# soedinglab/MMseqs2

Measured on AMD Instinct MI355X. Metric: sw_gcells_per_s, higher is better.
Workload: dtype int16

## Files before the change

### mmseqs2_amd/csrc/sw_body.h

```cpp
#pragma once
#include "mmgpu_internal.h"
#include "pf_device.h"

namespace mmgpu {

namespace {

constexpr int GROUP = 16;
constexpr int WAVES = 4;
constexpr int GROUPS_PER_WAVE = 64 / GROUP;
constexpr int HITS_PER_WAVE = 2 * GROUPS_PER_WAVE;
constexpr unsigned NEG2 = 0x80008000u;

typedef short s16x2 __attribute__((ext_vector_type(2)));
typedef unsigned short u16x2 __attribute__((ext_vector_type(2)));

__device__ __forceinline__ unsigned pk_add_sat(unsigned a, unsigned b) {
    return __builtin_bit_cast(unsigned, __builtin_elementwise_add_sat(__builtin_bit_cast(s16x2, a),
                                                                      __builtin_bit_cast(s16x2, b)));
}
__device__ __forceinline__ unsigned pk_max_s(unsigned a, unsigned b) {
    return __builtin_bit_cast(unsigned, __builtin_elementwise_max(__builtin_bit_cast(s16x2, a),
                                                                  __builtin_bit_cast(s16x2, b)));
}
__device__ __forceinline__ unsigned pk_max_u(unsigned a, unsigned b) {
    return __builtin_bit_cast(unsigned, __builtin_elementwise_max(__builtin_bit_cast(u16x2, a),
                                                                  __builtin_bit_cast(u16x2, b)));
}
__device__ __forceinline__ unsigned pk_sub_sat_u(unsigned a, unsigned b) {
    return __builtin_bit_cast(unsigned, __builtin_elementwise_sub_sat(__builtin_bit_cast(u16x2, a),
                                                                      __builtin_bit_cast(u16x2, b)));
}
__device__ __forceinline__ unsigned bfi(unsigned mask, unsigned a, unsigned b) {
    return (a & mask) | (b & ~mask);
}

constexpr int SW_HALF_LIMIT = 2048 - 256;
constexpr int SW_HALF_MAX_GAP = 2048;
constexpr int SW_HALF_MARK = -1;
typedef _Float16 h16x2 __attribute__((ext_vector_type(2)));
__device__ __forceinline__ h16x2 as_h(unsigned a) { return __builtin_bit_cast(h16x2, a); }
__device__ __forceinline__ unsigned as_u(h16x2 a) { return __builtin_bit_cast(unsigned, a); }
__device__ __forceinline__ unsigned h_add(unsigned a, unsigned b) { return as_u(as_h(a) + as_h(b)); }
__device__ __forceinline__ unsigned h_sub(unsigned a, unsigned b) { return as_u(as_h(a) - as_h(b)); }
__device__ __forceinline__ unsigned h_max(unsigned a, unsigned b) {
    return as_u(__builtin_elementwise_maximum(as_h(a), as_h(b)));
}
__device__ __forceinline__ unsigned h_max3(unsigned a, unsigned b, unsigned c) {
    return as_u(__builtin_elementwise_maximum(__builtin_elementwise_maximum(as_h(a), as_h(b)), as_h(c)));
}
__device__ __forceinline__ unsigned short h_bits(int v) { return __builtin_bit_cast(unsigned short, (_Float16)v); }
__device__ __forceinline__ int h_value(unsigned bits) { return (int)(float)__builtin_bit_cast(_Float16, (unsigned short)bits); }
__device__ __forceinline__ unsigned from_lane_above(unsigned head, unsigned v) {
    return __builtin_amdgcn_update_dpp(head, v, 0x111 , 0xF, 0xF, false);
}
__device__ __forceinline__ unsigned from_lane_above_or_zero(unsigned v) {
    return __builtin_amdgcn_update_dpp(0u, v, 0x111 , 0xF, 0xF, true);
}

#ifndef MMGPU_SW_PREFETCH
#define MMGPU_SW_PREFETCH 1
#endif
#define SW_KEEP_IN_ROW(x) asm volatile("" : "+v"(x))

template <int R>
struct Tile {
    static constexpr int ROWS = GROUP * R;
    static constexpr int LANE_STRIDE = lane_stride_bytes(R);
    static constexpr int ROW_STRIDE = GROUP * LANE_STRIDE;
};
static_assert(GROUP == 16, "sw_profile_bytes and sw_tiles (mmgpu_internal.h) assume 16-lane groups");

template <int R, bool REV, bool HALF = false>
__device__ __forceinline__ void build_profile(unsigned char *lds, const uint8_t *q, const int8_t *cb, int qlen,
                                              int tile_base, const int8_t *mat, int alphabet, const int8_t *prof) {
    using T = Tile<R>;
    const int total = (alphabet + 1) * T::ROWS;
    for (int idx = threadIdx.x; idx < total; idx += blockDim.x) {
        const int letter = idx / T::ROWS;
        const int row = idx - letter * T::ROWS;
        const int rg = tile_base + row;
        short v = (short)-32768;
        if (letter < alphabet && rg < qlen) {
            const int qi = REV ? (qlen - 1 - rg) : rg;
            v = prof ? (short)prof[letter * qlen + qi] : (short)((int)mat[letter * alphabet + q[qi]] + (int)cb[qi]);
        }
        const int lane = row / R, r = row - lane * R;
        if constexpr (HALF) v = (short)h_bits(v);
        *reinterpret_cast<short *>(lds + letter * T::ROW_STRIDE + lane * T::LANE_STRIDE + r * 2) = v;
    }
}

__device__ __forceinline__ bool sw_rev_wanted(const SwLaunch &L, uint32_t slot, int min_start) {
    const mmgpu_sw_hit &f = L.out[slot];
    const int s = f.score;
    if (L.rev_mode == 2) return s > 0 && L.rev_force[slot] != 0;
    return s > 0 && s >= min_start && !(L.rev_mode == 1 && f.word != 0);
}

constexpr int SW_REV_JOB_HITS = 1024;
static_assert(SW_REV_JOB_HITS == SW_REV_JOB_MAX, "host and kernel disagree on the reverse job size");
static_assert(SW_LDS_HEADER == SW_REV_JOB_HITS * 2 + 64, "the header holds the live hits and the scheduling words");
constexpr int SW_HALF_FLAG_AT = SW_REV_JOB_HITS * 2 + 20;
__device__ __forceinline__ uint32_t sw_half_any_marked() {
    extern __shared__ __attribute__((aligned(16))) unsigned char lds_all[];
    return *reinterpret_cast<const uint32_t *>(lds_all + SW_HALF_FLAG_AT);
}

template <int R, bool MULTI, bool REV, bool PF, bool HALF = false, bool MARKED = false>
__device__ __forceinline__ void sw_body(const SwLaunch &L, const SwJob job) {
    static_assert(!(HALF || MARKED) || (!MULTI && !REV && !(HALF && MARKED)), "f16 and its int16 re-run: single-tile forward scans");
    constexpr bool PACKED = REV || MARKED;
    using T = Tile<R>;
    extern __shared__ __attribute__((aligned(16))) unsigned char lds_all[];
    uint16_t *live = reinterpret_cast<uint16_t *>(lds_all);
    uint32_t *live_wave = reinterpret_cast<uint32_t *>(lds_all + SW_REV_JOB_HITS * 2);
    uint32_t *next_chunk = reinterpret_cast<uint32_t *>(lds_all + SW_REV_JOB_HITS * 2 + 16);
    uint32_t *half_flag = reinterpret_cast<uint32_t *>(lds_all + SW_HALF_FLAG_AT);
    unsigned char *lds = lds_all + SW_LDS_HEADER;
    if (MULTI) __builtin_amdgcn_s_setprio(3);
    const int lane = threadIdx.x & 63;
    const int wave = __builtin_amdgcn_readfirstlane(threadIdx.x >> 6);
    const int g = lane & (GROUP - 1);
    const int grp = lane / GROUP;

    const uint32_t qbeg = L.q_off[job.query];
    const int qlen = (int)(L.q_off[job.query + 1] - qbeg);
    const uint8_t *q = L.q_res + qbeg;
    const int8_t *cb = L.q_cb + qbeg;
    const int qbias = L.q_bias[job.query];
    const int8_t *prof = nullptr;
    if (L.q_prof_off) {
        const uint32_t po = L.q_prof_off[job.query];
        if (po != 0xFFFFFFFFu) prof = L.q_prof + po;
    }
    const int n_tiles = MULTI ? (int)sw_tiles((uint32_t)qlen, R) : 1;
    const uint32_t tile_bytes = sw_profile_bytes(R, L.alphabet);
    const bool resident = MULTI && sw_multi_resident((uint32_t)n_tiles, R, L.alphabet, L.resident_lds);
    const bool dynamic = !MULTI || resident;
    auto build_all_tiles = [&]() {
        for (int tile = 0; tile < n_tiles; ++tile)
            build_profile<R, REV>(lds + (uint32_t)tile * tile_bytes, q, cb, qlen, tile * T::ROWS, L.mat, L.alphabet, prof);
        __syncthreads();
    };

    const unsigned go2 = (HALF ? (unsigned)h_bits(L.gap_open) : (unsigned)L.gap_open) * 0x10001u;
    const unsigned ge2 = (HALF ? (unsigned)h_bits(L.gap_extend) : (unsigned)L.gap_extend) * 0x10001u;
    const unsigned pad_letter = (unsigned)L.alphabet;

    if (threadIdx.x == 0) *next_chunk = 0;
    if (HALF && threadIdx.x == 0) *half_flag = 0;
    if (!MULTI && !PACKED) {
        build_profile<R, REV, HALF>(lds, q, cb, qlen, 0, L.mat, L.alphabet, prof);
        __syncthreads();
    }
    if (MULTI && !REV && resident) build_all_tiles();

    uint32_t n_hits = job.hit_end - job.hit_begin;
    if (PACKED) {
        const int min_start = REV ? L.q_minstart[job.query] : 0;
        uint32_t total = 0;
        for (uint32_t base = 0; base < n_hits; base += WAVES * 64) {
            const uint32_t idx = base + threadIdx.x;
            bool pass = false;
            if (idx < n_hits) {
                const uint32_t slot = L.hit_out[job.hit_begin + idx];
                pass = MARKED ? L.out[slot].score == SW_HALF_MARK : sw_rev_wanted(L, slot, min_start);
            }
            const unsigned long long bal = __ballot(pass);
            if (lane == 0) live_wave[wave] = (uint32_t)__popcll(bal);
            __syncthreads();
            uint32_t before = 0, round_total = 0;
#pragma unroll
            for (int w = 0; w < WAVES; ++w) {
                const uint32_t c = live_wave[w];
                before += w < wave ? c : 0u;
                round_total += c;
            }
            if (pass) live[total + before + (uint32_t)__popcll(bal & ((1ull << lane) - 1ull))] = (uint16_t)idx;
            total += round_total;
            __syncthreads();
        }
        n_hits = total;
        if (n_hits == 0) return;
        if (!MULTI) {
            build_profile<R, REV>(lds, q, cb, qlen, 0, L.mat, L.alphabet, prof);
            __syncthreads();
        }
        if (MULTI && resident) build_all_tiles();
    }
    const uint32_t n_iter = (n_hits + WAVES * HITS_PER_WAVE - 1) / (WAVES * HITS_PER_WAVE);

    for (uint32_t it = 0; dynamic || it < n_iter; ++it) {
        uint32_t chunk = it * WAVES + wave;
        if (dynamic) {
            if (lane == 0) chunk = atomicAdd(next_chunk, 1u);
            chunk = __builtin_amdgcn_readfirstlane(chunk);
        }
        const uint32_t slot0 = chunk * HITS_PER_WAVE;
        if (dynamic && slot0 >= n_hits) break;

        const uint32_t sA = slot0 + grp * 2, sB = sA + 1;
        const bool vA = sA < n_hits, vB = sB < n_hits;
        const uint32_t hA = job.hit_begin + (PACKED ? (uint32_t)live[vA ? sA : 0] : sA);
        const uint32_t hB = job.hit_begin + (PACKED ? (uint32_t)live[vB ? sB : 0] : sB);
        const uint32_t tA = vA ? L.hit_target[hA] : 0u, tB = vB ? L.hit_target[hB] : 0u;
        const uint8_t *pA = L.t_res + (size_t)L.t_off4[tA] * 4;
        const uint8_t *pB = L.t_res + (size_t)L.t_off4[tB] * 4;
        int colsA = vA ? (int)L.t_len[tA] : 0, colsB = vB ? (int)L.t_len[tB] : 0;
        int r0A = 0, r0B = 0;
        int endA = 0, endB = 0;
        unsigned rev_target = 0xFFFFFFFFu;
        if (REV) {
            mmgpu_sw_hit fa, fb;
            fa.score = 0; fa.q_end = 0; fa.t_end = 0;
            fb = fa;
            if (vA) fa = L.out[L.hit_out[hA]];
            if (vB) fb = L.out[L.hit_out[hB]];
            colsA = vA ? fa.t_end + 1 : 0;
            colsB = vB ? fb.t_end + 1 : 0;
            endA = colsA > 0 ? fa.t_end : 0;
            endB = colsB > 0 ? fb.t_end : 0;
            r0A = colsA > 0 ? qlen - 1 - fa.q_end : 0;
            r0B = colsB > 0 ? qlen - 1 - fb.q_end : 0;
            rev_target = (colsA > 0 ? (unsigned)fa.score & 0xFFFFu : 0xFFFFu) | ((colsB > 0 ? (unsigned)fb.score & 0xFFFFu : 0xFFFFu) << 16);
        }
        int ncols = colsA > colsB ? colsA : colsB;
        ncols = max(ncols, __shfl_xor(ncols, 16));
        ncols = max(ncols, __shfl_xor(ncols, 32));
        ncols = __builtin_amdgcn_readfirstlane(ncols);
        const int nsteps = ncols + GROUP - 1;
        int mincols = colsA < colsB ? colsA : colsB;
        mincols = min(mincols, __shfl_xor(mincols, 16));
        mincols = min(mincols, __shfl_xor(mincols, 32));
        mincols = __builtin_amdgcn_readfirstlane(mincols);

        unsigned long long bestA = 0, bestB = 0;

        uint2 *scr = nullptr;
        unsigned scr_grp = 0;
        if (MULTI) {
            scr = L.scratch + (size_t)((job.shape >> 8) * WAVES + wave) * GROUPS_PER_WAVE * 2 * L.scratch_cols;
            scr_grp = (unsigned)grp * 2u * L.scratch_cols;
        }

        for (int tile = 0; tile < n_tiles; ++tile) {
            const int tile_base = tile * T::ROWS;
            if (MULTI && !resident) {
                __syncthreads();
                build_profile<R, REV>(lds, q, cb, qlen, tile_base, L.mat, L.alphabet, prof);
                __syncthreads();
            }
            const unsigned char *const lds_tile = MULTI && resident ? lds + (uint32_t)tile * tile_bytes : lds;
            const uint2 *scr_in = MULTI ? scr + (size_t)((tile + 1) & 1) * L.scratch_cols : nullptr;
            uint2 *scr_out = MULTI ? scr + (size_t)(tile & 1) * L.scratch_cols : nullptr;
            const bool has_above = MULTI && tile > 0;
            const bool has_below = MULTI && tile + 1 < n_tiles;

            unsigned Hp[R], E[R], aux[R];
#pragma unroll
            for (int r = 0; r < R; ++r) { Hp[r] = 0; E[r] = 0; aux[r] = 0; }
            if (REV) {
#pragma unroll
                for (int r = 0; r < R; ++r) {
                    const int rg = tile_base + g * R + r;
                    aux[r] = (rg >= r0A ? 0xFFFFu : 0u) | (rg >= r0B ? 0xFFFF0000u : 0u);
                }
            }
            unsigned vmax = 0, bestcol = 0xFFFFFFFFu;
            unsigned rev_rowA = 0, rev_rowB = 0;
            unsigned Hup_prev = 0;
            unsigned out_H = 0, out_F = 0;

            auto letters4 = [&](const uint8_t *p, int end, int k) -> unsigned {
                if (!REV) return reinterpret_cast<const unsigned *>(p)[k];
                int o = end - 3 - 4 * k;
                o = o < -3 ? -3 : o;
                unsigned w;
                __builtin_memcpy(&w, p + o, 4);
                return w;
            };
            unsigned wA = letters4(pA, endA, 0), wB = letters4(pB, endB, 0);
            unsigned wA_next = letters4(pA, endA, 1), wB_next = letters4(pB, endB, 1);
            uint2 bnd = make_uint2(0, 0), bnd_next = make_uint2(0, 0);
            auto boundary16 = [&](int m) -> uint2 {
                const int last = ncols - 1 < 0 ? 0 : ncols - 1;
                return scr_in[scr_grp + (unsigned)min(16 * m + g - (m > 0 ? 1 : 0), last)];
            };
            if (has_above) {
                bnd = boundary16(0);
                bnd_next = boundary16(1);
            }

            constexpr int ND = (R + 1) / 2;
            unsigned pav_next[PF ? ND : 1], pbv_next[PF ? ND : 1];
            auto load_rows = [&](unsigned letters, unsigned *pav, unsigned *pbv) {
                const unsigned a = letters & 0xFFu, b = (letters >> 8) & 0xFFu;
                const uint4 *rowA = reinterpret_cast<const uint4 *>(lds_tile + a * T::ROW_STRIDE + g * T::LANE_STRIDE);
                const uint4 *rowB = reinterpret_cast<const uint4 *>(lds_tile + b * T::ROW_STRIDE + g * T::LANE_STRIDE);
#pragma unroll
                for (int k = 0; k < ND / 4; ++k) {
                    const uint4 pa = rowA[k], pb = rowB[k];
                    pav[4 * k] = pa.x; pav[4 * k + 1] = pa.y; pav[4 * k + 2] = pa.z; pav[4 * k + 3] = pa.w;
                    pbv[4 * k] = pb.x; pbv[4 * k + 1] = pb.y; pbv[4 * k + 2] = pb.z; pbv[4 * k + 3] = pb.w;
                }
                if constexpr (ND % 4 >= 2) {
                    const uint2 pa = *reinterpret_cast<const uint2 *>(rowA + ND / 4);
                    const uint2 pb = *reinterpret_cast<const uint2 *>(rowB + ND / 4);
                    pav[(ND / 4) * 4] = pa.x; pav[(ND / 4) * 4 + 1] = pa.y;
                    pbv[(ND / 4) * 4] = pb.x; pbv[(ND / 4) * 4 + 1] = pb.y;
                }
                if constexpr (ND % 2 == 1) {
                    pav[ND - 1] = reinterpret_cast<const unsigned *>(rowA)[ND - 1];
                    pbv[ND - 1] = reinterpret_cast<const unsigned *>(rowB)[ND - 1];
                }
            };
            unsigned let = pad_letter * 0x101u;
            constexpr bool LETTER_BLOCKS = MULTI || REV || R >= 7;
            constexpr bool LETTER_QUEUE = !MULTI && R < 7;
            unsigned long long lq = 0;
            auto letter_block = [&](int k) {
                if (!LETTER_BLOCKS) return;
                unsigned a = wA, b = wB;
                if (4 * k + 4 > mincols) {
                    const unsigned pad4 = pad_letter * 0x01010101u;
                    const int na = min(max(colsA - 4 * k, 0), 4), nb = min(max(colsB - 4 * k, 0), 4);
                    const unsigned ma = REV ? ~(unsigned)(0xFFFFFFFFull >> (8 * na)) : (unsigned)((1ull << (8 * na)) - 1ull);
                    const unsigned mb = REV ? ~(unsigned)(0xFFFFFFFFull >> (8 * nb)) : (unsigned)((1ull << (8 * nb)) - 1ull);
                    a = bfi(ma, a, pad4);
                    b = bfi(mb, b, pad4);
                }
                const unsigned lo = __builtin_amdgcn_perm(b, a, REV ? 0x06020703u : 0x05010400u);
                const unsigned hi = __builtin_amdgcn_perm(b, a, REV ? 0x04000501u : 0x07030602u);
                lq = ((unsigned long long)hi << 32) | lo;
            };
            auto head_letters = [&](int c, int j) -> unsigned {
                if (LETTER_BLOCKS && LETTER_QUEUE) { const unsigned v = (unsigned)lq; lq >>= 16; return v; }
                if (LETTER_BLOCKS) return (unsigned)(lq >> (16 * j));
                const unsigned sh = (unsigned)(REV ? 3 - j : j) * 8u;
                const unsigned la0 = __builtin_amdgcn_ubfe(wA, sh, 8u);
                const unsigned lb0 = __builtin_amdgcn_ubfe(wB, sh, 8u);
                return (c < colsA ? la0 : pad_letter) | ((c < colsB ? lb0 : pad_letter) << 8);
            };
            letter_block(0);
            let = from_lane_above(head_letters(0, 0), let);
            if (PF) load_rows(let, pav_next, pbv_next);

            for (int s0 = -1; s0 < nsteps; s0 += 4) {
            if (MULTI && s0 > 0 && ((s0 + 1) & 15) == 0) {
                bnd = bnd_next;
                if (has_above) bnd_next = boundary16(((s0 + 1) >> 4) + 1);
            }
            const int jn = min(4, nsteps - s0);
#pragma nounroll
            for (int j = s0 < 0 ? 1 : 0; j < jn; ++j) {
                const int s = s0 + j;
                if (has_below && s >= GROUP) {
                    if (g == GROUP - 1) (scr_out + (s - GROUP))[scr_grp] = make_uint2(out_H, out_F);
                }
                const unsigned Hup = MULTI ? from_lane_above(bnd.x, out_H) : from_lane_above_or_zero(out_H);
                unsigned f = MULTI ? from_lane_above(bnd.y, out_F) : from_lane_above_or_zero(out_F);
                if (MULTI) {
                    bnd.x = __builtin_amdgcn_update_dpp(bnd.x, bnd.x, 0x12F, 0xF, 0xF, false);
                    bnd.y = __builtin_amdgcn_update_dpp(bnd.y, bnd.y, 0x12F, 0xF, 0xF, false);
                }
                unsigned pav[ND], pbv[ND];
                if (PF) {
#pragma unroll
                    for (int k = 0; k < ND; ++k) { pav[k] = pav_next[k]; pbv[k] = pbv_next[k]; }
                } else {
                    load_rows(let, pav, pbv);
                }

                unsigned hd = Hup_prev;
                Hup_prev = Hup;
                unsigned cmax = 0;
                unsigned pre[R], es[R];
#pragma unroll
                for (int r = 0; r < R; ++r) {
                    unsigned P = __builtin_amdgcn_perm(pbv[r / 2], pav[r / 2], (r & 1) ? 0x07060302u : 0x05040100u);
                    if (REV) P = __builtin_amdgcn_bitop3_b32(aux[r], P, NEG2, 0xCA);
                    if constexpr (HALF) {
                        pre[r] = h_add(r == 0 ? hd : Hp[r - 1], P);
                        es[r] = h_sub(E[r], ge2);
                    } else {
                        pre[r] = pk_max_s(pk_add_sat(r == 0 ? hd : Hp[r - 1], P), E[r]);
                        es[r] = pk_sub_sat_u(E[r], ge2);
                    }
                }
                let = from_lane_above(head_letters(s + 1, j), let);
                if (PF) load_rows(let, pav_next, pbv_next);
#pragma unroll
                for (int r = 0; r < R; ++r) {
                    unsigned h;
                    if constexpr (HALF) {
                        h = h_max3(pre[r], E[r], f);
                        const unsigned fs = h_sub(f, ge2);
                        const unsigned t = h_sub(h, go2);
                        cmax = r == 0 ? h : h_max(cmax, h);
                        f = h_max3(fs, t, 0u);
                        E[r] = h_max3(es[r], t, 0u);
                    } else {
                        h = pk_max_s(pre[r], f);
                        const unsigned fs = pk_sub_sat_u(f, ge2);
                        const unsigned t = pk_sub_sat_u(h, go2);
                        cmax = pk_max_u(cmax, h);
                        f = pk_max_u(fs, t);
                        E[r] = pk_max_u(es[r], t);
                    }
                    SW_KEEP_IN_ROW(E[r]);
                    Hp[r] = h;
                }
                out_H = Hp[R - 1];
                out_F = f;

                const int col = s - g;

                const unsigned nm = pk_max_u(vmax, cmax);
                if (nm != vmax) {
                    const unsigned diff = nm ^ vmax;
                    if (!REV) {
                        const unsigned mask = ((diff & 0xFFFFu) ? 0xFFFFu : 0u) | ((diff >> 16) ? 0xFFFF0000u : 0u);
                        bestcol = bfi(mask, ((unsigned)col & 0xFFFFu) * 0x10001u, bestcol);
#pragma unroll
                        for (int r = 0; r < R; ++r) aux[r] = bfi(mask, Hp[r], aux[r]);
                    } else {
                        const unsigned x = nm ^ rev_target;
                        const bool hitA = (diff & 0xFFFFu) && !(x & 0xFFFFu), hitB = (diff >> 16) && !(x >> 16);
                        if (hitA | hitB) {
                            asm volatile("" ::: "memory");
                            unsigned ra = 0, rb = 0;
#pragma unroll
                            for (int r = R - 1; r >= 0; --r) {
                                if ((Hp[r] & 0xFFFFu) == (rev_target & 0xFFFFu)) ra = (unsigned)r;
                                if ((Hp[r] >> 16) == (rev_target >> 16)) rb = (unsigned)r;
                            }
                            if (hitA) { bestcol = (bestcol & 0xFFFF0000u) | ((unsigned)col & 0xFFFFu); rev_rowA = ra; }
                            if (hitB) { bestcol = (bestcol & 0xFFFFu) | ((unsigned)col << 16); rev_rowB = rb; }
                        }
                    }
                    vmax = nm;
                }
            }
            {
                wA = wA_next; wB = wB_next;
                const int k = ((s0 + 1) >> 2) + 2;
                wA_next = letters4(pA, endA, k); wB_next = letters4(pB, endB, k);
                letter_block(k - 1);
            }
            }
            if (has_below && ncols > 0 && g == GROUP - 1) (scr_out + (ncols - 1))[scr_grp] = make_uint2(out_H, out_F);

            unsigned rowA_first = rev_rowA, rowB_first = rev_rowB;
            unsigned sA = vmax & 0xFFFFu, sB = vmax >> 16;
            if (!REV) {
#pragma unroll
                for (int r = R - 1; r >= 0; --r) {
                    if ((aux[r] & 0xFFFFu) == sA) rowA_first = (unsigned)r;
                    if ((aux[r] >> 16) == sB) rowB_first = (unsigned)r;
                }
            } else {
                sA = sA == (rev_target & 0xFFFFu) ? sA : 0u;
                sB = sB == (rev_target >> 16) ? sB : 0u;
            }
            const unsigned rgA = (unsigned)(tile_base + g * R) + rowA_first;
            const unsigned rgB = (unsigned)(tile_base + g * R) + rowB_first;
            unsigned long long keyA = sA ? ((unsigned long long)sA << 32) | ((0xFFFFu - (bestcol & 0xFFFFu)) << 16) | (0xFFFFu - rgA) : 0ull;
            unsigned long long keyB = sB ? ((unsigned long long)sB << 32) | ((0xFFFFu - (bestcol >> 16)) << 16) | (0xFFFFu - rgB) : 0ull;
#pragma unroll
            for (int m = 1; m < GROUP; m <<= 1) {
                const unsigned long long oa = __shfl_xor(keyA, m), ob = __shfl_xor(keyB, m);
                keyA = oa > keyA ? oa : keyA;
                keyB = ob > keyB ? ob : keyB;
            }
            bestA = keyA > bestA ? keyA : bestA;
            bestB = keyB > bestB ? keyB : bestB;
        }

        if (g == 0) {
#pragma unroll
            for (int half = 0; half < 2; ++half) {
                const bool valid = half ? vB : vA;
                if (!valid) continue;
                const unsigned long long key = half ? bestB : bestA;
                const uint32_t h = half ? hB : hA;
                const bool marked = HALF && (unsigned)(key >> 32) > (unsigned)h_bits(SW_HALF_LIMIT);
                const int score = HALF ? (marked ? SW_HALF_MARK : h_value((unsigned)(key >> 32))) : (int)(key >> 32);
                const int col = 0xFFFF - (int)((key >> 16) & 0xFFFFu);
                const int row = 0xFFFF - (int)(key & 0xFFFFu);
                mmgpu_sw_hit *o = L.out + L.hit_out[h];
                if (!REV) {
                    mmgpu_sw_hit res;
                    res.score = score;
                    res.q_end = score ? row : 0;
                    res.t_end = score ? col : -1;
                    res.q_start = -1;
                    res.t_start = -1;
                    res.word = (score + qbias >= 255) ? 1 : 0;
                    *o = res;
                    if (marked) *half_flag = 1;
                } else {
                    const int end = half ? endB : endA;
                    const int cols = half ? colsB : colsA;
                    if (cols > 0) {
                        o->t_start = (score == o->score) ? end - col : -2;
                        o->q_start = (score == o->score) ? qlen - 1 - row : -2;
                    }
                }
            }
        }
    }
}

template <int R, bool MULTI, bool BOTH>
__device__ __forceinline__ void sw_passes(const SwLaunch &L, const SwJob &job) {
    if constexpr (R <= SW_MAX_R) {
        constexpr bool PF = MMGPU_SW_PREFETCH && !MULTI && (BOTH || R <= 24);
        if (!(BOTH && L.rev_only)) sw_body<R, MULTI, false, PF>(L, job);
        if constexpr (BOTH && !MULTI) {
            __threadfence_block();
            __syncthreads();
            sw_body<R, MULTI, true, PF>(L, job);
        }
    }
}

#ifndef MMGPU_SW_WAVES_G0F
#define MMGPU_SW_WAVES_G0F 4
#endif
#ifndef MMGPU_SW_WAVES_G0B
#define MMGPU_SW_WAVES_G0B 2
#endif
#ifndef MMGPU_SW_WAVES_G1F
#define MMGPU_SW_WAVES_G1F 3
#endif
#ifndef MMGPU_SW_WAVES_G1B
#define MMGPU_SW_WAVES_G1B 2
#endif

}

}
```

### mmseqs2_amd/csrc/sw_half_kernel.hip

```cpp
#include "mmgpu_internal.h"
#include "pf_device.h"
#include "sw_body.h"

namespace mmgpu {

namespace {

template <int R, bool BOTH>
__device__ __forceinline__ void sw_half_passes(const SwLaunch &L, const SwJob &job) {
    if constexpr (R <= SW_MAX_R) {
        constexpr bool PF = MMGPU_SW_PREFETCH && (BOTH || R <= 24);
        sw_body<R, false, false, PF, true, false>(L, job);
        __threadfence_block();
        __syncthreads();
        if (sw_half_any_marked()) {
            sw_body<R, false, false, PF, false, true>(L, job);
            __threadfence_block();
            __syncthreads();
        }
        if constexpr (BOTH) sw_body<R, false, true, PF>(L, job);
    }
}

constexpr bool SW_HALF_FORWARD_ONLY[3] = {false, false, false};

template <int G, bool BOTH>
__global__ __launch_bounds__(WAVES * 64)
__attribute__((amdgpu_waves_per_eu(G == 0 ? (BOTH ? MMGPU_SW_WAVES_G0B : MMGPU_SW_WAVES_G0F)
                                           : (G == 1 ? (BOTH ? MMGPU_SW_WAVES_G1B : MMGPU_SW_WAVES_G1F) : SW_MIN_WAVES),
                                   G == 1 && BOTH ? MMGPU_SW_WAVES_G1B : 8))) void sw_half_kernel(SwLaunch L) {
    SwJob job = L.jobs[blockIdx.x];
    if (L.q_hit_count) {
        const uint32_t lim = job.query * L.hit_stride + L.q_hit_count[job.query];
        job.hit_end = job.hit_end < lim ? job.hit_end : lim;
        if (job.hit_end <= job.hit_begin) return;
    }
#define MMGPU_SW_SINGLE(R) case (R) - 1: sw_half_passes<R, BOTH>(L, job); break;
    if constexpr (G == 0) {
        switch (job.shape & 0xFFu) {
            MMGPU_SW_SINGLE(1) MMGPU_SW_SINGLE(2) MMGPU_SW_SINGLE(3) MMGPU_SW_SINGLE(4) MMGPU_SW_SINGLE(5) MMGPU_SW_SINGLE(6)
            MMGPU_SW_SINGLE(7) MMGPU_SW_SINGLE(8) MMGPU_SW_SINGLE(9) MMGPU_SW_SINGLE(10) MMGPU_SW_SINGLE(11) MMGPU_SW_SINGLE(12)
            default: break;
        }
    } else if constexpr (G == 1) {
        switch (job.shape & 0xFFu) {
            MMGPU_SW_SINGLE(13) MMGPU_SW_SINGLE(14) MMGPU_SW_SINGLE(15) MMGPU_SW_SINGLE(16) MMGPU_SW_SINGLE(17) MMGPU_SW_SINGLE(18)
            MMGPU_SW_SINGLE(19) MMGPU_SW_SINGLE(20) MMGPU_SW_SINGLE(21) MMGPU_SW_SINGLE(22) MMGPU_SW_SINGLE(23) MMGPU_SW_SINGLE(24)
            default: break;
        }
    } else {
        switch (job.shape & 0xFFu) {
            MMGPU_SW_SINGLE(25) MMGPU_SW_SINGLE(26) MMGPU_SW_SINGLE(27) MMGPU_SW_SINGLE(28) MMGPU_SW_SINGLE(29) MMGPU_SW_SINGLE(30)
            MMGPU_SW_SINGLE(31) MMGPU_SW_SINGLE(32)
            default: break;
        }
    }
#undef MMGPU_SW_SINGLE
}

#ifdef MMGPU_SW_HALF_AUDIT_FORWARD
template __global__ void sw_half_kernel<0, false>(SwLaunch);
template __global__ void sw_half_kernel<1, false>(SwLaunch);
template __global__ void sw_half_kernel<2, false>(SwLaunch);
#endif

}

bool launch_sw_half(const SwLaunch &L, int group, size_t lds_bytes, bool both_passes, hipStream_t stream) {
    if (group < 0 || group > 2 || (group == 2 && SW_GROUPS != 4)) return false;
    if (!both_passes && !SW_HALF_FORWARD_ONLY[group]) return false;
    dim3 grid(L.n_jobs), block(WAVES * 64);
    const size_t lds = lds_bytes + SW_LDS_HEADER;
    switch (group) {
        case 0: hipLaunchKernelGGL((sw_half_kernel<0, true>), grid, block, lds, stream, L); break;
        case 1: hipLaunchKernelGGL((sw_half_kernel<1, true>), grid, block, lds, stream, L); break;
        default: hipLaunchKernelGGL((sw_half_kernel<2, true>), grid, block, lds, stream, L); break;
    }
    return true;
}

void warm_sw_half() {
    hipFuncAttributes a;
    (void)hipFuncGetAttributes(&a, reinterpret_cast<const void *>(&sw_half_kernel<0, true>));
}

}
```

Measured before the change: 4926.

## Run reverse SW pass in packed f16 with int16 fallback on overflow

```diff
diff --git a/mmseqs2_amd/csrc/sw_body.h b/mmseqs2_amd/csrc/sw_body.h
--- a/mmseqs2_amd/csrc/sw_body.h
+++ b/mmseqs2_amd/csrc/sw_body.h
@@ -11,6 +11,7 @@
 constexpr int GROUPS_PER_WAVE = 64 / GROUP;
 constexpr int HITS_PER_WAVE = 2 * GROUPS_PER_WAVE;
 constexpr unsigned NEG2 = 0x80008000u;
+constexpr unsigned NEG2_HALF = 0xF800F800u;
 
 typedef short s16x2 __attribute__((ext_vector_type(2)));
 typedef unsigned short u16x2 __attribute__((ext_vector_type(2)));
@@ -108,8 +109,8 @@
 }
 
 template <int R, bool MULTI, bool REV, bool PF, bool HALF = false, bool MARKED = false>
-__device__ __forceinline__ void sw_body(const SwLaunch &L, const SwJob job) {
-    static_assert(!(HALF || MARKED) || (!MULTI && !REV && !(HALF && MARKED)), "f16 and its int16 re-run: single-tile forward scans");
+__device__ __forceinline__ bool sw_body(const SwLaunch &L, const SwJob job) {
+    static_assert(!(HALF || MARKED) || (!MULTI && !(MARKED && REV) && !(HALF && MARKED)), "f16 and its int16 re-run: single-tile scans");
     constexpr bool PACKED = REV || MARKED;
     using T = Tile<R>;
     extern __shared__ __attribute__((aligned(16))) unsigned char lds_all[];
@@ -117,6 +118,7 @@
     uint32_t *live_wave = reinterpret_cast<uint32_t *>(lds_all + SW_REV_JOB_HITS * 2);
     uint32_t *next_chunk = reinterpret_cast<uint32_t *>(lds_all + SW_REV_JOB_HITS * 2 + 16);
     uint32_t *half_flag = reinterpret_cast<uint32_t *>(lds_all + SW_HALF_FLAG_AT);
+    uint32_t *over_wave = reinterpret_cast<uint32_t *>(lds_all + SW_REV_JOB_HITS * 2 + 24);
     unsigned char *lds = lds_all + SW_LDS_HEADER;
     if (MULTI) __builtin_amdgcn_s_setprio(3);
     const int lane = threadIdx.x & 63;
@@ -149,7 +151,7 @@
     const unsigned pad_letter = (unsigned)L.alphabet;
 
     if (threadIdx.x == 0) *next_chunk = 0;
-    if (HALF && threadIdx.x == 0) *half_flag = 0;
+    if (HALF && !REV && threadIdx.x == 0) *half_flag = 0;
     if (!MULTI && !PACKED) {
         build_profile<R, REV, HALF>(lds, q, cb, qlen, 0, L.mat, L.alphabet, prof);
         __syncthreads();
@@ -160,15 +162,21 @@
     if (PACKED) {
         const int min_start = REV ? L.q_minstart[job.query] : 0;
         uint32_t total = 0;
+        uint32_t any_over = 0;
         for (uint32_t base = 0; base < n_hits; base += WAVES * 64) {
             const uint32_t idx = base + threadIdx.x;
-            bool pass = false;
+            bool pass = false, over = false;
             if (idx < n_hits) {
                 const uint32_t slot = L.hit_out[job.hit_begin + idx];
                 pass = MARKED ? L.out[slot].score == SW_HALF_MARK : sw_rev_wanted(L, slot, min_start);
+                if constexpr (REV && HALF) over = pass && L.out[slot].score > SW_HALF_LIMIT;
             }
             const unsigned long long bal = __ballot(pass);
             if (lane == 0) live_wave[wave] = (uint32_t)__popcll(bal);
+            if constexpr (REV && HALF) {
+                const unsigned long long obal = __ballot(over);
+                if (lane == 0) over_wave[wave] = obal != 0ull ? 1u : 0u;
+            }
             __syncthreads();
             uint32_t before = 0, round_total = 0;
 #pragma unroll
@@ -176,15 +184,17 @@
                 const uint32_t c = live_wave[w];
                 before += w < wave ? c : 0u;
                 round_total += c;
+                if constexpr (REV && HALF) any_over |= over_wave[w];
             }
             if (pass) live[total + before + (uint32_t)__popcll(bal & ((1ull << lane) - 1ull))] = (uint16_t)idx;
             total += round_total;
             __syncthreads();
         }
         n_hits = total;
-        if (n_hits == 0) return;
+        if (n_hits == 0) return true;
+        if (REV && HALF && any_over) return false;
         if (!MULTI) {
-            build_profile<R, REV>(lds, q, cb, qlen, 0, L.mat, L.alphabet, prof);
+            build_profile<R, REV, HALF>(lds, q, cb, qlen, 0, L.mat, L.alphabet, prof);
             __syncthreads();
         }
         if (MULTI && resident) build_all_tiles();
@@ -223,7 +233,9 @@
             endB = colsB > 0 ? fb.t_end : 0;
             r0A = colsA > 0 ? qlen - 1 - fa.q_end : 0;
             r0B = colsB > 0 ? qlen - 1 - fb.q_end : 0;
-            rev_target = (colsA > 0 ? (unsigned)fa.score & 0xFFFFu : 0xFFFFu) | ((colsB > 0 ? (unsigned)fb.score & 0xFFFFu : 0xFFFFu) << 16);
+            const unsigned tgA = HALF ? (unsigned)h_bits(fa.score) : (unsigned)fa.score & 0xFFFFu;
+            const unsigned tgB = HALF ? (unsigned)h_bits(fb.score) : (unsigned)fb.score & 0xFFFFu;
+            rev_target = (colsA > 0 ? tgA : 0xFFFFu) | ((colsB > 0 ? tgB : 0xFFFFu) << 16);
         }
         int ncols = colsA > colsB ? colsA : colsB;
         ncols = max(ncols, __shfl_xor(ncols, 16));
@@ -379,10 +391,10 @@
 #pragma unroll
                 for (int r = 0; r < R; ++r) {
                     unsigned P = __builtin_amdgcn_perm(pbv[r / 2], pav[r / 2], (r & 1) ? 0x07060302u : 0x05040100u);
-                    if (REV) P = __builtin_amdgcn_bitop3_b32(aux[r], P, NEG2, 0xCA);
+                    if (REV) P = __builtin_amdgcn_bitop3_b32(aux[r], P, HALF ? NEG2_HALF : NEG2, 0xCA);
                     if constexpr (HALF) {
                         pre[r] = h_add(r == 0 ? hd : Hp[r - 1], P);
-                        es[r] = h_sub(E[r], ge2);
+                        if constexpr (!REV) es[r] = h_sub(E[r], ge2);
                     } else {
                         pre[r] = pk_max_s(pk_add_sat(r == 0 ? hd : Hp[r - 1], P), E[r]);
                         es[r] = pk_sub_sat_u(E[r], ge2);
@@ -399,7 +411,7 @@
                         const unsigned t = h_sub(h, go2);
                         cmax = r == 0 ? h : h_max(cmax, h);
                         f = h_max3(fs, t, 0u);
-                        E[r] = h_max3(es[r], t, 0u);
+                        E[r] = h_max3(REV ? h_sub(E[r], ge2) : es[r], t, 0u);
                     } else {
                         h = pk_max_s(pre[r], f);
                         const unsigned fs = pk_sub_sat_u(f, ge2);
@@ -484,7 +496,7 @@
                 if (!valid) continue;
                 const unsigned long long key = half ? bestB : bestA;
                 const uint32_t h = half ? hB : hA;
-                const bool marked = HALF && (unsigned)(key >> 32) > (unsigned)h_bits(SW_HALF_LIMIT);
+                const bool marked = HALF && !REV && (unsigned)(key >> 32) > (unsigned)h_bits(SW_HALF_LIMIT);
                 const int score = HALF ? (marked ? SW_HALF_MARK : h_value((unsigned)(key >> 32))) : (int)(key >> 32);
                 const int col = 0xFFFF - (int)((key >> 16) & 0xFFFFu);
                 const int row = 0xFFFF - (int)(key & 0xFFFFu);
@@ -510,6 +522,7 @@
             }
         }
     }
+    return true;
 }
 
 template <int R, bool MULTI, bool BOTH>
diff --git a/mmseqs2_amd/csrc/sw_half_kernel.hip b/mmseqs2_amd/csrc/sw_half_kernel.hip
--- a/mmseqs2_amd/csrc/sw_half_kernel.hip
+++ b/mmseqs2_amd/csrc/sw_half_kernel.hip
@@ -5,6 +5,11 @@
 namespace mmgpu {
 
 namespace {
+
+#ifndef MMGPU_SW_REV_HALF
+#define MMGPU_SW_REV_HALF 1
+#endif
+constexpr int SW_REV_HALF_MIN_R = 1;
 
 template <int R, bool BOTH>
 __device__ __forceinline__ void sw_half_passes(const SwLaunch &L, const SwJob &job) {
@@ -18,7 +23,12 @@
             __threadfence_block();
             __syncthreads();
         }
-        if constexpr (BOTH) sw_body<R, false, true, PF>(L, job);
+        if constexpr (BOTH) {
+            if constexpr (MMGPU_SW_REV_HALF && R >= SW_REV_HALF_MIN_R) {
+                if (sw_body<R, false, true, PF, true>(L, job)) return;
+            }
+            sw_body<R, false, true, PF>(L, job);
+        }
     }
 }
 
```

Result: no change. 4966, median of 6 (+0.8%).
